# rtqichen/torchdiffeq

Measured on AMD Instinct MI355X. Metric: dopri5 RK-stages/sec at batch=65536x dim=128 (end-to-end adaptive trial steps incl. func, error norm, read-back and hos~, higher is better.
Workload: dtype f32; 1 GPU; BASELINE.json configs[1]: dopri5 adaptive, linear ODE dy/dt=Ay, batch=65536 x dim=128 fp32 per GPU, rtol=1e-7 atol=1e-9; global_batch=65536, rows_per_gpu=65536, dim=128, parallelism=batch-sharded x1, accepted=1937, rejected=2, lookahead=True, hip_graph=False

## Files before the change

### include/tdeq_hip.h

```cpp
#ifndef TDEQ_HIP_H
#define TDEQ_HIP_H

#include <stddef.h>
#include <stdint.h>

#ifdef __cplusplus
extern "C" {
#endif

#define TDEQ_ABI_VERSION 33
#define TDEQ_F32 0
#define TDEQ_F64 1
#define TDEQ_C64 2
#define TDEQ_C128 3
#define TDEQ_BF16 4
#define TDEQ_F16 5
#define TDEQ_MAX_TERMS 14
#define TDEQ_MAX_SUM_TERMS 8
#define TDEQ_MAX_DENSE_OUTPUTS 16
#define TDEQ_MAX_SEGMENTS 4096
#define TDEQ_INLINE_SEGMENTS 16
#define TDEQ_CHUNK_QUANTUM 1024

#define TDEQ_EINVAL (-1)
#define TDEQ_EWORKSPACE (-2)
// ... 78 lines not shown
int tdeq_stage_combine_multi_dev(const tdeq_multi_out* outs, int n_out, const void* y0, const void* acc_in,
                                 const void* const* k, int n_terms, const double* ctrl_dev, int64_t n, int dtype,
                                 void* stream);
int tdeq_stage_combine_multi_timed(const tdeq_multi_out* outs, int n_out, const void* y0, const void* acc_in,
                                   const void* const* k, int n_terms, double dt, int64_t n, int dtype, void* stream,
                                   void* start_event, void* stop_event);

int tdeq_error_norm_partial_ctrl(const void* err_partial, const void* y0, const void* y1, const void* const* k,
                                 const double* coef, int n_terms, double dt, const tdeq_segment* segs,
                                 const void* segs_dev, int n_seg, int64_t chunk, int64_t n_chunks, double* out_sumsq,
                                 double* out_nonfinite, const tdeq_step_ctrl* ctrl, double* out_ctrl, double* ctrl_dev,
                                 void* next_times, int state_in_dev, void* copy_last_k, void* workspace,
                                 size_t workspace_bytes, int dtype, void* stream);
int tdeq_stage_combine_sel(void* out, const void* y_acc, const void* f_acc, const void* y_rej, const void* f_rej,
                           double coef, const double* ctrl_dev, int64_t n, int dtype, void* stream);

int tdeq_step_controller(const double* sums, const double* nonfinite, const tdeq_segment* segs, const void* segs_dev,
                         int n_seg, double* out_sumsq, double* out_nonfinite, const tdeq_step_ctrl* ctrl,
                         double* out_ctrl, double* ctrl_dev, void* next_times, int state_in_dev, int dtype,
                         void* stream);

int tdeq_stage_combine_dev(void* out, void* err_out, const void* y0, const void* const* k, const double* coef,
                           const double* err_coef, int n_terms, const double* ctrl_dev, int64_t n, int dtype,
                           void* stream);
int tdeq_step_commit(void* y_prev, void* f_prev, void* y_cur, void* f_cur, const void* y1, const void* f1,
                     const double* ctrl_dev, int64_t n, int dtype, void* stream);

int tdeq_init_norms(int mode, const void* a, const void* b, const void* yscale,
                    const tdeq_segment* segs, const void* segs_dev, int n_seg, int64_t chunk,
                    int64_t n_chunks, double* out_sumsq, double* out_nonfinite, void* workspace, size_t workspace_bytes,
// ... 198 lines not shown
```

### torchdiffeq_amd/_native.py

```python
from __future__ import annotations

import contextlib
import ctypes
import functools
import math
import os
import threading
from typing import List, Optional, Sequence, Tuple

import numpy as np
import torch

TDEQ_ABI_VERSION = 33
TDEQ_F32, TDEQ_F64 = 0, 1
TDEQ_C64, TDEQ_C128 = 2, 3
TDEQ_BF16, TDEQ_F16 = 4, 5
TDEQ_MAX_TERMS = 14
TDEQ_INLINE_SEGMENTS = 16
TDEQ_CHUNK_QUANTUM = 1024
TDEQ_MAX_STAGE_TIMES = 16
TDEQ_MAX_DENSE_OUTPUTS = 16
TDEQ_MAX_MULTI_OUT = 4
TDEQ_MAX_GATHER = 4

_LIB_NAME = "libtdeq_hip.so"
_LIB_PATH = os.path.join(os.path.dirname(os.path.abspath(__file__)), _LIB_NAME)

_c_void_pp = ctypes.POINTER(ctypes.c_void_p)
# ... 104 lines not shown
                                                    ctypes.c_void_p, ctypes.c_int, ctypes.c_void_p, ctypes.c_void_p, ctypes.c_size_t,
                                                    ctypes.c_int, ctypes.c_void_p]),
    "tdeq_step_controller": (ctypes.c_int, [ctypes.c_void_p, ctypes.c_void_p, ctypes.POINTER(Segment), ctypes.c_void_p,
                                            ctypes.c_int, ctypes.c_void_p, ctypes.c_void_p,
                                            ctypes.POINTER(StepCtrl), ctypes.c_void_p, ctypes.c_void_p,
                                            ctypes.c_void_p, ctypes.c_int, ctypes.c_int, ctypes.c_void_p]),
    "tdeq_stage_combine_dev": (ctypes.c_int, [ctypes.c_void_p, ctypes.c_void_p, ctypes.c_void_p, _c_void_pp,
                                              _c_double_p, _c_double_p, ctypes.c_int, ctypes.c_void_p, ctypes.c_int64,
                                              ctypes.c_int, ctypes.c_void_p]),
    "tdeq_step_commit": (ctypes.c_int, [ctypes.c_void_p, ctypes.c_void_p, ctypes.c_void_p, ctypes.c_void_p,
                                        ctypes.c_void_p, ctypes.c_void_p, ctypes.c_void_p, ctypes.c_int64,
                                        ctypes.c_int, ctypes.c_void_p]),
    "tdeq_stage_combine_sel": (ctypes.c_int, [ctypes.c_void_p, ctypes.c_void_p, ctypes.c_void_p, ctypes.c_void_p,
                                              ctypes.c_void_p, ctypes.c_double, ctypes.c_void_p, ctypes.c_int64,
                                              ctypes.c_int, ctypes.c_void_p]),
    "tdeq_init_norms": (ctypes.c_int, [ctypes.c_int, ctypes.c_void_p, ctypes.c_void_p, ctypes.c_void_p,
                                       ctypes.POINTER(Segment), ctypes.c_void_p, ctypes.c_int,
                                       ctypes.c_int64, ctypes.c_int64, ctypes.c_void_p, ctypes.c_void_p,
                                       ctypes.c_void_p, ctypes.c_size_t, ctypes.c_int, ctypes.c_void_p]),
    "tdeq_init_scaled": (ctypes.c_int, [ctypes.c_int, ctypes.c_void_p, ctypes.c_void_p, ctypes.c_void_p,
                                        ctypes.POINTER(Segment), ctypes.c_void_p, ctypes.c_int, ctypes.c_int64,
                                        ctypes.c_int64, ctypes.c_void_p, ctypes.c_void_p, ctypes.c_int,
                                        ctypes.c_void_p]),
    "tdeq_dense_eval": (ctypes.c_int, [ctypes.c_void_p, ctypes.c_void_p, ctypes.c_void_p, ctypes.c_void_p,
                                       ctypes.c_void_p, _c_void_pp, _c_double_p, ctypes.c_int,
                                       ctypes.c_double, ctypes.c_double, ctypes.c_int64, ctypes.c_int,
                                       ctypes.c_void_p]),
    "tdeq_dense_eval_multi": (ctypes.c_int, [ctypes.c_void_p, ctypes.c_int64, ctypes.c_void_p, ctypes.c_void_p,
                                             ctypes.c_void_p, ctypes.c_void_p, _c_void_pp, _c_double_p, ctypes.c_int,
                                             ctypes.c_double, _c_double_p, ctypes.c_int, ctypes.c_int64, ctypes.c_int,
# ... 499 lines not shown
                                               dtype_code(y0.dtype), self._stream()), "tdeq_stage_combine_dev")

    def step_commit(self, y_prev, f_prev, y_cur, f_cur, y1, f1, plan: NormPlan) -> None:
        _check(self.lib.tdeq_step_commit(y_prev.data_ptr(), f_prev.data_ptr(), y_cur.data_ptr(), f_cur.data_ptr(),
                                         y1.data_ptr(), f1.data_ptr(), plan.ctrl_dev.data_ptr(), y_cur.numel(),
                                         dtype_code(y_cur.dtype), self._stream()), "tdeq_step_commit")

    def arm_readback(self, plan: NormPlan, n_sum: int = 1, ctrl: bool = True) -> None:
        self._arm(plan, n_sum, ctrl=ctrl)

    def stage_combine_sel(self, out, y_acc, f_acc, y_rej, f_rej, coef: float, plan: NormPlan) -> None:
        _check(self.lib.tdeq_stage_combine_sel(out.data_ptr(), y_acc.data_ptr(), f_acc.data_ptr(), y_rej.data_ptr(),
                                               f_rej.data_ptr(), coef, plan.ctrl_dev.data_ptr(), out.numel(),
                                               dtype_code(out.dtype), self._stream()), "tdeq_stage_combine_sel")

    def dense_eval(self, out, y0, y1, f0, f1, ks, coefs, dt: float, x: float) -> None:
        ptrs, cf, n = self._terms(ks, coefs)
        _check(self.lib.tdeq_dense_eval(out.data_ptr(), y0.data_ptr(), y1.data_ptr(), f0.data_ptr(),
                                        f1.data_ptr(), ptrs, cf, n, dt, x, y0.numel(),
                                        dtype_code(y0.dtype), self._stream()), "tdeq_dense_eval")

    def dense_eval_multi(self, out_rows, y0, y1, f0, f1, ks, coefs, dt: float, xs: Sequence[float]) -> None:
        ptrs, cf, n = self._terms(ks, coefs)
        m = len(xs)
        xa = (ctypes.c_double * m)(*xs)
        _check(self.lib.tdeq_dense_eval_multi(out_rows.data_ptr(), out_rows.stride(0) if m > 1 else y0.numel(),
                                              y0.data_ptr(), y1.data_ptr(), f0.data_ptr(), f1.data_ptr(), ptrs, cf, n,
                                              dt, xa, m, y0.numel(), dtype_code(y0.dtype), self._stream()),
               "tdeq_dense_eval_multi")

# ... 545 lines not shown
```

### torchdiffeq_amd/csrc/tdeq_abi.hip

```cpp
#include <hip/hip_runtime.h>
#include <hip/hip_ext.h>

#include <cstdlib>

#include "tdeq_kernels.hpp"
#include "tdeq_kernels_complex.hpp"
#include "tdeq_kernels_lp.hpp"

namespace {
using namespace tdeq;

constexpr int64_t kMaxGrid = 1 << 16;

inline unsigned stream_grid(int64_t n_items, int items_per_block) {
    int64_t g = (n_items + items_per_block - 1) / items_per_block;
    const int64_t cap = kMaxGrid;
    if (g > cap) g = cap;
    if (g < 1) g = 1;
    return (unsigned)g;
}

inline bool aligned16(const void* p) { return (reinterpret_cast<uintptr_t>(p) & 15u) == 0; }

inline int check_launch() {
// ... 530 lines not shown
    const bool vec = aligned16(out) && aligned16(y_acc) && aligned16(f_acc) && aligned16(y_rej) && aligned16(f_rej);
    if (vec) {
        const dim3 g(stream_grid(n / L, kBlock)), b(kBlock);
        switch (stream_policy((int64_t)3 * n * (int64_t)sizeof(T))) {
            case 1: hipLaunchKernelGGL((stage_combine_sel_kernel<T, true, 1>), g, b, 0, s, a); break;
            case 2: hipLaunchKernelGGL((stage_combine_sel_kernel<T, true, 2>), g, b, 0, s, a); break;
            case 3: hipLaunchKernelGGL((stage_combine_sel_kernel<T, true, 3>), g, b, 0, s, a); break;
            default: hipLaunchKernelGGL((stage_combine_sel_kernel<T, true, 0>), g, b, 0, s, a);
        }
    } else {
        hipLaunchKernelGGL((stage_combine_sel_kernel<T, false>), dim3(stream_grid(n, kBlock)), dim3(kBlock), 0, s, a);
    }
    return check_launch();
}

template <typename T>
int launch_init(int mode, const void* a_, const void* b_, const void* y_, const SegTable& st,
                double* out_sumsq, double* out_bad, double* ws, hipStream_t s) {
    InitArgs<T> a;
    a.a = static_cast<const T*>(a_);
    a.b = static_cast<const T*>(b_);
    a.y = static_cast<const T*>(y_);
    a.st = st;
    a.part0 = ws;
    a.part1 = ws + st.n_chunks;
    a.part_bad = ws + 2 * st.n_chunks;
    const bool vec = aligned16(a_) && aligned16(b_) && aligned16(y_);
    const dim3 g((unsigned)st.n_chunks), b(kBlock);
    if (mode == 0) {
        if (vec) hipLaunchKernelGGL((init_norms_kernel<T, 0, true>), g, b, 0, s, a);
// ... 777 lines not shown
    return dtype == TDEQ_F32 ? launch_commit<float>(y_prev, f_prev, y_cur, f_cur, y1, f1, ctrl_dev, n, s)
                             : launch_commit<double>(y_prev, f_prev, y_cur, f_cur, y1, f1, ctrl_dev, n, s);
}

int tdeq_stage_combine_sel(void* out, const void* y_acc, const void* f_acc, const void* y_rej, const void* f_rej,
                           double coef, const double* ctrl_dev, int64_t n, int dtype, void* stream) {
    if (!out || !y_acc || !f_acc || !y_rej || !f_rej || !ctrl_dev || n < 0 || (bad_dtype(dtype) && !lp_dtype(dtype))) return TDEQ_EINVAL;
    if (n == 0) return 0;
    hipStream_t s = static_cast<hipStream_t>(stream);
    if (dtype == TDEQ_BF16) return lp_launch_sel<lp::BF16>(out, y_acc, f_acc, y_rej, f_rej, coef, ctrl_dev, n, s);
    if (dtype == TDEQ_F16) return lp_launch_sel<lp::F16>(out, y_acc, f_acc, y_rej, f_rej, coef, ctrl_dev, n, s);
    return dtype == TDEQ_F32 ? launch_combine_sel<float>(out, y_acc, f_acc, y_rej, f_rej, coef, ctrl_dev, n, s)
                             : launch_combine_sel<double>(out, y_acc, f_acc, y_rej, f_rej, coef, ctrl_dev, n, s);
}

int tdeq_init_norms(int mode, const void* a, const void* b, const void* yscale, const tdeq_segment* segs,
                    const void* segs_dev, int n_seg, int64_t chunk, int64_t n_chunks, double* out_sumsq,
                    double* out_nonfinite, void* workspace, size_t workspace_bytes, int dtype,
                    void* stream) {
    if ((mode != 0 && mode != 1) || !a || !b || !yscale || !out_sumsq || !out_nonfinite || !workspace ||
        (bad_norm_dtype(dtype) && !lp_dtype(dtype)))
        return TDEQ_EINVAL;
    SegTable st;
    const int e = fill_segtable(st, segs, segs_dev, n_seg, chunk, n_chunks);
    if (e) return e;
    if (workspace_bytes < tdeq_workspace_bytes(n_chunks)) return TDEQ_EWORKSPACE;
    hipStream_t s = static_cast<hipStream_t>(stream);
    double* ws = static_cast<double*>(workspace);
    if (dtype == TDEQ_BF16) return lp_launch_init<lp::BF16>(mode, a, b, yscale, st, out_sumsq, out_nonfinite, ws, nullptr, nullptr, s);
    if (dtype == TDEQ_F16) return lp_launch_init<lp::F16>(mode, a, b, yscale, st, out_sumsq, out_nonfinite, ws, nullptr, nullptr, s);
// ... 323 lines not shown
```

### torchdiffeq_amd/csrc/tdeq_kernels.hpp

```cpp
#pragma once

#include <hip/hip_runtime.h>
#include <stdint.h>

#include "tdeq_hip.h"

namespace tdeq {

constexpr int kBlock = 256;
constexpr int kWave = 64;

typedef float f32x4 __attribute__((ext_vector_type(4)));
typedef double f64x2 __attribute__((ext_vector_type(2)));

template <typename T> struct VecOf;
template <> struct VecOf<float> { using type = f32x4; static constexpr int L = 4; };
template <> struct VecOf<double> { using type = f64x2; static constexpr int L = 2; };

template <typename V> __device__ __forceinline__ V vabs(V v);
template <> __device__ __forceinline__ f32x4 vabs(f32x4 v) {
    return f32x4{__builtin_fabsf(v.x), __builtin_fabsf(v.y), __builtin_fabsf(v.z), __builtin_fabsf(v.w)};
}
template <> __device__ __forceinline__ f64x2 vabs(f64x2 v) {
    return f64x2{__builtin_fabs(v.x), __builtin_fabs(v.y)};
// ... 230 lines not shown
            multi_elem<T, NT, E, POLICY, NOUTC, ACCC, DEVDT>(a, i);
    }
    if (VEC) {
        const int64_t t = ne * L + threadIdx.x;
        if (blockIdx.x == 0 && t < a.n) multi_elem<T, NT, T>(a, t);
    }
}

__device__ __forceinline__ double wave_sum(double v) {
#pragma unroll
    for (int off = kWave / 2; off > 0; off >>= 1) v += __shfl_down(v, off, kWave);
    return v;
}

template <int NV>
__device__ __forceinline__ void block_sum(double (&v)[NV], double* red) {
    const int lane = threadIdx.x & (kWave - 1);
    const int wave = threadIdx.x / kWave;
#pragma unroll
    for (int q = 0; q < NV; ++q) {
        v[q] = wave_sum(v[q]);
        if (lane == 0) red[q * (kBlock / kWave) + wave] = v[q];
    }
    __syncthreads();
    if (threadIdx.x == 0) {
#pragma unroll
        for (int q = 0; q < NV; ++q) {
            double s = red[q * (kBlock / kWave)];
#pragma unroll
            for (int w = 1; w < kBlock / kWave; ++w) s += red[q * (kBlock / kWave) + w];
            v[q] = s;
        }
    }
}

struct SegTable {
    tdeq_segment inl[TDEQ_INLINE_SEGMENTS];
    const tdeq_segment* dev;
    int n_seg;
    int64_t chunk;
    int64_t n_chunks;
};

__device__ __forceinline__ tdeq_segment get_segment(const SegTable& st, int s) {
    if (st.n_seg <= TDEQ_INLINE_SEGMENTS) return st.inl[s];
    return st.dev[s];
}

// ... 528 lines not shown
    float tt;
    if ((c.alpha_is_one >> i) & 1u) tt = ctl_prev16(t1T, tkind);
    else tt = ctl_rnd16(t0T + ctl_rnd16((float)c.alpha[i] * dtT, tkind), tkind);
    return ctl_bits16((float)c.time_sign * tt, tkind);
}

template <typename T>
__device__ __forceinline__ T ctl_stage_time(const tdeq_step_ctrl& c, double t0n, double dtn, int i) {
    const T t0T = (T)t0n, dtT = (T)dtn, t1T = (T)(t0n + dtn);
    T tt;
    if ((c.alpha_is_one >> i) & 1u) tt = ctl_prev(t1T);
    else tt = t0T + (T)c.alpha[i] * dtT;
    return (T)c.time_sign * tt;
}

constexpr int kCtrlInlineSegments = 4;
template <int NS>
__global__ __launch_bounds__(kBlock) void norm_finalize_ctrl_kernel(const CtrlArgs a) {
    __shared__ double red[2 * NS * (kBlock / kWave)];
    __shared__ double seg_val[2][NS];
    __shared__ double next_step[2];
    const int n_seg = a.st.n_seg;
    if (a.presummed) {
        const double* sums = a.in_sumsq ? a.in_sumsq : a.out_sumsq;
        if (a.in_sumsq)
            for (int s = threadIdx.x; s < n_seg; s += kBlock) {
                a.out_sumsq[s] = a.in_sumsq[s];
                a.out_bad[s] = a.in_bad[s];
            }
        double part[2] = {0.0, 0.0};
// ... 69 lines not shown
    if (threadIdx.x == 0) {
        const double dev_t0 = a.ctrl_dev[2], dev_dt = a.ctrl_dev[3];
        const double arg_t0 = c.t0, arg_dt = c.dt;
        const double step_t0 = a.state_in_dev ? dev_t0 : arg_t0;
        const double step_dt = a.state_in_dev ? dev_dt : arg_dt;
        double val = 0.0;
        if (a.presummed) val = seg_val[0][0];
        for (int s = 0; s < c.n_norm_seg && s < n_seg && !a.presummed; ++s) {
            const int64_t numel = a.st.inl[s].numel;
            if (numel == 0) continue;
            const double v = (s == 0 && numel == 1 && c.leading_abs && a.ratio_kind >= 2)
                                 ? (double)ctl_rnd16((float)seg_val[0][s], a.ratio_kind)
                                 : ctl_seg_norm(seg_val[0][s], numel, a.ratio_kind);
            val = ctl_nan_max(val, v);
        }
        const double ratio = a.ratio_kind == 1 ? (double)(float)val : val;
        bool accept = ratio <= 1.0;
        if (step_dt > c.max_step) accept = false;
        if (step_dt <= c.min_step) accept = true;
        double dt_next;
        if (ratio == 0.0) {
            dt_next = step_dt * c.ifactor;
        } else {
            const double dfactor = ratio < 1.0 ? 1.0 : c.dfactor;
            const double scaled = c.safety / pow(ratio, c.exponent);
            dt_next = step_dt * ctl_nan_min(c.ifactor, ctl_nan_max(scaled, dfactor));
        }
        dt_next = ctl_clamp(dt_next, c.min_step, c.max_step);
        const double t0n = accept ? step_t0 + step_dt : step_t0;
        double dtn = dt_next;
        if (!__builtin_isfinite(dtn)) dtn = c.min_step;
        dtn = ctl_clamp(dtn, c.min_step, c.max_step);
        a.ctrl_dev[0] = accept ? 1.0 : 0.0;
        a.ctrl_dev[1] = ctl_round_T(dtn, a.is_f32) * c.time_sign;
        a.ctrl_dev[2] = t0n;
        a.ctrl_dev[3] = dtn;
        next_step[0] = t0n;
        next_step[1] = dtn;
        a.out_ctrl[0] = accept ? 1.0 : 0.0;
        a.out_ctrl[1] = dt_next;
        a.out_ctrl[2] = ratio;
        a.out_ctrl[3] = t0n;
    }
    __syncthreads();
    const int i = threadIdx.x;
    if (i < c.n_times) {
        if (a.is_f32 >= 2) static_cast<uint16_t*>(a.next_times)[i] = ctl_stage_time16(c, next_step[0], next_step[1], i, a.is_f32);
        else if (a.is_f32) static_cast<float*>(a.next_times)[i] = ctl_stage_time<float>(c, next_step[0], next_step[1], i);
        else static_cast<double*>(a.next_times)[i] = ctl_stage_time<double>(c, next_step[0], next_step[1], i);
    }
    if (i < n_seg && !a.presummed) {
        a.out_sumsq[i] = seg_val[0][i];
        a.out_bad[i] = seg_val[1][i];
    }
}

template <typename T>
struct CombineDevArgs {
    T* out;
    T* err_out;
    const T* y0;
    const T* k[TDEQ_MAX_TERMS];
    T c[TDEQ_MAX_TERMS];
    T e[TDEQ_MAX_TERMS];
    int nt;
// ... 169 lines not shown
    const E* __restrict__ y = reinterpret_cast<const E*>(ys);
    const E* __restrict__ f = reinterpret_cast<const E*>(fs);
    if (i0 < ne) {
        if (!accept) {
            y_spec = ld_stream<POLICY>(y + i0);
            f_spec = ld_stream<POLICY>(f + i0);
        }
        st_stream<POLICY>(out + i0, y_spec + f_spec * c);
    }
    for (int64_t i = i0 + stride; i < ne; i += stride)
        st_stream<POLICY>(out + i, ld_stream<POLICY>(y + i) + ld_stream<POLICY>(f + i) * c);
    if (VEC) {
        const int64_t t = ne * L + threadIdx.x;
        if (blockIdx.x == 0 && t < a.n) a.out[t] = ys[t] + fs[t] * c;
    }
}

template <typename T, int NT>
struct DenseArgs {
    T* out;
    const T* y0;
    const T* y1;
    const T* f0;
    const T* f1;
    const T* k[NT];
    T c[NT];
    T dt;
    T x;
    int64_t n;
};
// ... 616 lines not shown
```

### torchdiffeq_amd/solvers/adaptive.py

```python
from __future__ import annotations

import bisect
import collections
import math
import os
import warnings
from typing import List, Optional, Sequence

import numpy as np
import torch

from .. import _native
from .._graph import (_AUTO_CAPTURE_AFTER_STEPS, _AUTO_MIN_GRID_STEPS, _GRAPH_AUTO_MAX_ELEMENTS,
                     _GRAPH_MODE_MAX_ELEMENTS, _CaptureFailed, _DtCell, _GraphStep, _capture, _graph_request,
                     _held_tensor_ptrs, _reusable_across_solves, _scalar_state, _side_effect_fingerprint, _side_stream,
                     _request_is_explicit, _stream_is_capturing, clear_graph_cache)
from .._scalars import is_low, power, rdiv, scalar_type
from ..autodiff import Ops, stitch
from ..misc import (BuiltinNorm, OdeFunc, Perturb, StateLayout, component_norm, find_event, handle_unused_kwargs, rms_norm,
                   vector_tolerances)
from ..misc import _null_callback as _null
from ..tableaus import (ADAPTIVE_HEUN, ADAPTIVE_TABLEAUS, BOSH3, CARRY_DEFAULT_ON, DOPRI5, DOPRI8, FEHLBERG2, FUSE_ODEINT, TSIT5, SparseRow,
                       Tableau, adams_coefficients, carry_plan, fused_lead, row_by_row_plan)
from ._common import _nan_max, _nan_min, _clamp, _norm_value, _as_float, optimal_step_size, optimal_step_size_in, _StepShadow, _NoShadow, _NO_SHADOW
from .events import AdaptiveEvents

STEP_CALLBACKS = ("callback_step", "callback_accept_step", "callback_reject_step")


class _LockStep:

    def __init__(self, group, replicated=()):
        import torch.distributed as dist
        self.dist = dist
        self.group = None if group is True else group
        self.replicated = sorted(set(int(i) for i in replicated))
        self.rank = dist.get_rank(self.group)
        backend = dist.get_backend(self.group)
        self.on_device = backend == "nccl"

# ... 183 lines not shown
            and func.time_dtype == y0.dtype and dist_sync is None
        device_ctrl = (getattr(self.kernels, "device_controller", True)
                       and (self._fuse is not None or self._whole_row_ctrl or self._vec_ctrl)
                       and (isinstance(self.norm, BuiltinNorm) or self._vec_ctrl)
                       and len(self._beta) <= _native.TDEQ_MAX_STAGE_TIMES and n_norm_seg >= 0
                       and self.step_t is None and self.jump_t is None and (self._sync is None or sync_dev)
                       and self._wide)
        self._plan_dev = self._plan_glob = None
        if device_ctrl and self._sync is not None:
            segs = self.layout.segments(rtol, atol)
            self._plan_dev = _native.NormPlan(segs, self.layout.total, self.layout.chunk, y0.device, pinned=False)
            self._plan_glob = self.kernels.make_plan([(off, gn, rt, at) for (off, _, rt, at), gn in
                                                      zip(segs, self._numels)], self.layout.total,
                                                     self.layout.chunk, y0.device)
        self._lookahead = device_ctrl and os.environ.get("TDEQ_LOOKAHEAD", "1") != "0"
        wanted, auto = _graph_request(hip_graph)
        self._graph_auto = auto
        self._graph_explicit = _request_is_explicit(hip_graph)
        if wanted and _stream_is_capturing():
            wanted = False
        self._graph_watch = wanted and auto and y0.device.type == "cuda"
        self._auto = None
        self._auto_steps = 0
        self._hold_pre = False
        self.hip_graph = wanted and device_ctrl and self._sync is None and y0.device.type == "cuda" \
            and (not self._vec_ctrl or getattr(self.kernels, "vec_ctrl_in_graph", False)) \
            and hasattr(self.kernels, "stage_combine_dev") \
            and self.layout.total <= (_GRAPH_AUTO_MAX_ELEMENTS if auto else _GRAPH_MODE_MAX_ELEMENTS) * \
            (2 if (y0.element_size() == 2 and not auto) else 1)
        if wanted and not auto and not self.hip_graph and hip_graph is not None:
# ... 473 lines not shown
        func, kern = self.func, self.kernels
        builtin_norm, vec_fused = self._partial_norm()
        ks, coefs = [k[j] for j in err_rem[0]], err_rem[1]
        vec_ctrl = self._vec_ctrl and not builtin_norm and (err_partial is None or vec_fused)
        if lookahead and ((err_partial is not None and (builtin_norm or vec_ctrl))
                          or (self._whole_row_ctrl and builtin_norm) or vec_ctrl):
            ctrl = self._ctrl
            ctrl.t0, ctrl.dt = t0, dt
            tnext = torch.empty(ctrl.n_times, dtype=func.time_dtype, device=y0.device)
            if vec_ctrl:
                kern.error_norm_vec_ctrl(self.plan, y0, y1, ks, coefs, dt_signed, self._vec_fused[0], self._vec_fused[1],
                                         ctrl, tnext, **({} if err_partial is None else {"partial": err_partial}))
            elif err_partial is None:
                kern.error_norm_ctrl(self.plan, y0, y1, ks, coefs, dt_signed, ctrl, tnext)
            elif self._sync is None:
                kern.error_norm_partial_ctrl(self.plan, err_partial, y0, y1, ks, coefs, dt_signed, ctrl, tnext)
            else:
                kern.error_norm_partial(self._plan_dev, err_partial, y0, y1, ks, coefs, dt_signed)
                self._sync.reduce_device(self._plan_dev.out, self.plan.n_seg)
                kern.step_controller(self.plan, self._plan_dev, self._plan_glob, ctrl, tnext, y0.dtype)
            if t1 < self._t_end and not self._hold_pre and not self._last_trial:
                yi_n = torch.empty_like(y0)
                kern.stage_combine_sel(yi_n, y1, k[-1], y0, f0, self._beta[0].coef[0], self.plan)
                tn = tnext.unbind(0)
                self._pre = (yi_n, tn, func.eval_at(tn[0], yi_n))
            accept_dev, dt_next_dev, error_ratio, bad = kern.read_ctrl(self.plan)
            return error_ratio, any(b != 0 for b in bad), (accept_dev, dt_next_dev)
        if not builtin_norm:
            return self._user_norm_ratio(y0, y1, k, dt_signed, err_partial, err_rem) + (None,)
        if err_partial is not None:
            kern.error_norm_partial(self.plan, err_partial, y0, y1, ks, coefs, dt_signed)
        else:
            kern.error_norm(self.plan, y0, y1, ks, coefs, dt_signed)
        sumsq, _, bad = self._read_norms()
        return self._segment_norm(sumsq, bad), any(b != 0 for b in bad), None

    def _commit(self, accept_step, dt_next, y0, y1, k, t0, dt, t1, dt_signed, dsh, dsh_signed, on_step_t, on_jump_t,
                y1_nonfinite) -> None:
        func = self.func
        if accept_step:
            if func.callback_accept_step is not _null:
                func.callback_accept_step(self._time_tensor(t0), y0, self._time_tensor(dt))
            rec = _DenseRecord(y0, y1, k, dt_signed, t0, t1, dsh_signed, self._anchor)
            if dsh is not None:
                clipped = on_step_t or on_jump_t
                self._anchor = None if clipped else (dsh if self._anchor is None else self._anchor + dsh)
                func.set_time_anchor(self._anchor)
            if on_step_t and self.next_step_index != len(self._step_t) - 1:
                self.next_step_index += 1
            f1 = k[-1]
# ... 109 lines not shown
```

Before: 17980 RK-stages/s.

## Fuse error norm, step controller and next-stage combine into one persistent kernel

Adds a single persistent-grid kernel that computes the error-norm partial sums, performs a grid-wide reduction through tagged atomic granules with spin-waiting, runs the step-size controller, and writes the selected next-stage input (accepted or rejected branch). This replaces the separate error_norm_partial_ctrl and stage_combine_sel launches and their extra passes over y0/y1/k. It is enabled automatically for large single-segment states. It relies on all workgroups being co-resident and falls back to the separate launches, with a warning, if a workgroup times out waiting.

Result: faster. 18410 RK-stages/s, median of 6 (+2.4%).

```diff
diff --git a/include/tdeq_hip.h b/include/tdeq_hip.h
--- a/include/tdeq_hip.h
+++ b/include/tdeq_hip.h
@@ -8,7 +8,7 @@
 extern "C" {
 #endif
 
-#define TDEQ_ABI_VERSION 33
+#define TDEQ_ABI_VERSION 34
 #define TDEQ_F32 0
 #define TDEQ_F64 1
 #define TDEQ_C64 2
@@ -117,6 +117,14 @@
                                  size_t workspace_bytes, int dtype, void* stream);
 int tdeq_stage_combine_sel(void* out, const void* y_acc, const void* f_acc, const void* y_rej, const void* f_rej,
                            double coef, const double* ctrl_dev, int64_t n, int dtype, void* stream);
+
+#define TDEQ_STEP_END_WORKSPACE_BYTES 8192
+int tdeq_step_end_fused(const void* err_partial, const void* y0, const void* y1, const void* const* k, const double* coef,
+                        int n_terms, double dt, const tdeq_segment* segs, int n_seg, int64_t chunk, int64_t n_chunks,
+                        double* out_sumsq, double* out_nonfinite, const tdeq_step_ctrl* ctrl, double* out_ctrl,
+                        double* ctrl_dev, void* next_times, void* out, const void* y_rej, const void* f_rej,
+                        double stage_coef, void* sync_workspace, size_t sync_workspace_bytes, int* status, int dtype,
+                        void* stream);
 
 int tdeq_step_controller(const double* sums, const double* nonfinite, const tdeq_segment* segs, const void* segs_dev,
                          int n_seg, double* out_sumsq, double* out_nonfinite, const tdeq_step_ctrl* ctrl,
diff --git a/torchdiffeq_amd/_native.py b/torchdiffeq_amd/_native.py
--- a/torchdiffeq_amd/_native.py
+++ b/torchdiffeq_amd/_native.py
@@ -11,7 +11,7 @@
 import numpy as np
 import torch
 
-TDEQ_ABI_VERSION = 33
+TDEQ_ABI_VERSION = 34
 TDEQ_F32, TDEQ_F64 = 0, 1
 TDEQ_C64, TDEQ_C128 = 2, 3
 TDEQ_BF16, TDEQ_F16 = 4, 5
@@ -146,6 +146,13 @@
     "tdeq_stage_combine_sel": (ctypes.c_int, [ctypes.c_void_p, ctypes.c_void_p, ctypes.c_void_p, ctypes.c_void_p,
                                               ctypes.c_void_p, ctypes.c_double, ctypes.c_void_p, ctypes.c_int64,
                                               ctypes.c_int, ctypes.c_void_p]),
+    "tdeq_step_end_fused": (ctypes.c_int, [ctypes.c_void_p, ctypes.c_void_p, ctypes.c_void_p, _c_void_pp, _c_double_p,
+                                           ctypes.c_int, ctypes.c_double, ctypes.POINTER(Segment), ctypes.c_int,
+                                           ctypes.c_int64, ctypes.c_int64, ctypes.c_void_p, ctypes.c_void_p,
+                                           ctypes.POINTER(StepCtrl), ctypes.c_void_p, ctypes.c_void_p, ctypes.c_void_p,
+                                           ctypes.c_void_p, ctypes.c_void_p, ctypes.c_void_p, ctypes.c_double,
+                                           ctypes.c_void_p, ctypes.c_size_t, ctypes.c_void_p, ctypes.c_int,
+                                           ctypes.c_void_p]),
     "tdeq_init_norms": (ctypes.c_int, [ctypes.c_int, ctypes.c_void_p, ctypes.c_void_p, ctypes.c_void_p,
                                        ctypes.POINTER(Segment), ctypes.c_void_p, ctypes.c_int,
                                        ctypes.c_int64, ctypes.c_int64, ctypes.c_void_p, ctypes.c_void_p,
@@ -675,6 +682,50 @@
                                                f_rej.data_ptr(), coef, plan.ctrl_dev.data_ptr(), out.numel(),
                                                dtype_code(out.dtype), self._stream()), "tdeq_stage_combine_sel")
 
+    step_end_fused_capable = True
+    STEP_END_WORKSPACE_BYTES = 8192
+
+    def step_end_fused(self, plan: NormPlan, err_partial, y0, y1, ks, coefs, dt: float, ctrl: StepCtrl, next_times,
+                       out, y_rej, f_rej, stage_coef: float) -> bool:
+        if getattr(plan, "step_end_ws", None) is None:
+            plan.step_end_ws = torch.zeros(self.STEP_END_WORKSPACE_BYTES // 8, dtype=torch.int64, device=y0.device)
+            plan.step_end_status = torch.zeros(4, dtype=torch.int32, device="cpu", pin_memory=True)
+            plan.step_end_status_np = plan.step_end_status.numpy()
+        n = len(ks)
+        ptrs = (ctypes.c_void_p * max(n, 1))(*[k.data_ptr() for k in ks])
+        cf = (ctypes.c_double * max(n, 1))(*coefs)
+        self._arm(plan, 1, ctrl=True)
+        rc = self.lib.tdeq_step_end_fused(
+            err_partial.data_ptr(), y0.data_ptr(), y1.data_ptr(), ptrs, cf, n, dt, plan.segs, plan.n_seg, plan.chunk,
+            plan.n_chunks, plan.out_ptr, plan.bad_ptr, ctypes.byref(ctrl), plan.ctrl_ptr, plan.ctrl_dev.data_ptr(),
+            next_times.data_ptr(), out.data_ptr(), y_rej.data_ptr(), f_rej.data_ptr(), stage_coef,
+            plan.step_end_ws.data_ptr(), self.STEP_END_WORKSPACE_BYTES, plan.step_end_status.data_ptr(),
+            dtype_code(y0.dtype), self._stream())
+        if rc in (-1, -2):
+            plan.expect = ()
+            return False
+        _check(rc, "tdeq_step_end_fused")
+        return True
+
+    def read_ctrl_fused(self, plan: NormPlan):
+        status = plan.step_end_status_np
+        if plan.pinned and self._mode == "poll" and plan.expect:
+            bits, sent = plan.out_bits, self._SENTINEL
+            (a0, a1), (b0, b1) = plan.expect
+            spins = 0
+            while ((bits[a0:a1] == sent).any() or (bits[b0:b1] == sent).any()) and status[0] == 0:
+                spins += 1
+                if spins & 0xFFFFF == 0:
+                    torch.cuda.current_stream().synchronize()
+                    break
+        else:
+            torch.cuda.current_stream().synchronize()
+        if status[0] != 0:
+            torch.cuda.current_stream().synchronize()
+            plan.expect = ()
+            return None
+        return self.read_ctrl(plan)
+
     def dense_eval(self, out, y0, y1, f0, f1, ks, coefs, dt: float, x: float) -> None:
         ptrs, cf, n = self._terms(ks, coefs)
         _check(self.lib.tdeq_dense_eval(out.data_ptr(), y0.data_ptr(), y1.data_ptr(), f0.data_ptr(),
diff --git a/torchdiffeq_amd/csrc/tdeq_abi.hip b/torchdiffeq_amd/csrc/tdeq_abi.hip
--- a/torchdiffeq_amd/csrc/tdeq_abi.hip
+++ b/torchdiffeq_amd/csrc/tdeq_abi.hip
@@ -568,6 +568,74 @@
     return check_launch();
 }
 
+constexpr long long kEndSpinTicks = 400000;
+
+inline int device_cu_count() {
+    int dev = 0, cus = 0;
+    if (hipGetDevice(&dev) != hipSuccess) return 0;
+    if (hipDeviceGetAttribute(&cus, hipDeviceAttributeMultiprocessorCount, dev) != hipSuccess) return 0;
+    return cus;
+}
+
+template <typename T>
+int step_end_geometry(const SegTable& st, const void* const* ptrs, int n_ptrs, int& vpl) {
+    constexpr int L = VecOf<T>::L;
+    if (st.n_seg != 1 || st.inl[0].chunk_start != 0) return TDEQ_EINVAL;
+    const int64_t numel = st.inl[0].numel;
+    if (numel < L || numel % L != 0 || numel > st.chunk * st.n_chunks) return TDEQ_EINVAL;
+    if (st.n_chunks != (numel + st.chunk - 1) / st.chunk) return TDEQ_EINVAL;
+    if (st.chunk % (L * kBlock) != 0) return TDEQ_EINVAL;
+    vpl = (int)(st.chunk / (L * kBlock));
+    if (vpl != 1 && vpl != 2) return TDEQ_EINVAL;
+    const int64_t capacity = (int64_t)kEndGrid * kEndQuarters * (kEndVecs / vpl);
+    if (st.n_chunks > capacity) return TDEQ_EINVAL;
+    for (int q = 0; q < n_ptrs; ++q) if (!aligned16(ptrs[q])) return TDEQ_EINVAL;
+    return 0;
+}
+
+template <typename T>
+int launch_step_end(const void* partial, const void* y0, const void* y1, const void* k_last, double coef_err, double dt,
+                    const SegTable& st, double* out_sumsq, double* out_bad, const tdeq_step_ctrl* ctrl, double* out_ctrl,
+                    double* ctrl_dev, void* next_times, void* out, const void* y_rej, const void* f_rej, double coef,
+                    void* sync_ws, int* status, hipStream_t s) {
+    const void* ptrs[7] = {partial, y0, y1, k_last, out, y_rej, f_rej};
+    int vpl = 0;
+    const int e = step_end_geometry<T>(st, ptrs, 7, vpl);
+    if (e) return e;
+    static const int cus = device_cu_count();
+    if (cus < kEndGrid) return TDEQ_EINVAL;
+    StepEndArgs<T> a;
+    a.partial = static_cast<const T*>(partial);
+    a.y0 = static_cast<const T*>(y0);
+    a.y1 = static_cast<const T*>(y1);
+    a.k_last = static_cast<const T*>(k_last);
+    a.c_err = (T)coef_err * (T)dt;
+    a.numel = st.inl[0].numel;
+    a.chunk = st.chunk;
+    a.n_chunks = st.n_chunks;
+    a.rtol = st.inl[0].rtol;
+    a.atol = st.inl[0].atol;
+    a.c = *ctrl;
+    a.tkind = sizeof(T) == 4 ? 1 : 0;
+    a.out_sumsq = out_sumsq;
+    a.out_bad = out_bad;
+    a.out_ctrl = out_ctrl;
+    a.ctrl_dev = ctrl_dev;
+    a.next_times = next_times;
+    a.out = static_cast<T*>(out);
+    a.y_rej = static_cast<const T*>(y_rej);
+    a.f_rej = static_cast<const T*>(f_rej);
+    a.coef = (T)coef;
+    a.granules = static_cast<unsigned long long*>(sync_ws);
+    a.ticket = reinterpret_cast<unsigned*>(a.granules + kEndGrid * kEndGranules);
+    a.status = status;
+    a.spin_ticks = kEndSpinTicks;
+    const dim3 g(kEndGrid), b(kEndBlock);
+    if (vpl == 2) hipLaunchKernelGGL((step_end_fused_kernel<T, 2>), g, b, 0, s, a);
+    else hipLaunchKernelGGL((step_end_fused_kernel<T, 1>), g, b, 0, s, a);
+    return check_launch();
+}
+
 template <typename T>
 int launch_init(int mode, const void* a_, const void* b_, const void* y_, const SegTable& st,
                 double* out_sumsq, double* out_bad, double* ws, hipStream_t s) {
@@ -1375,6 +1443,31 @@
                              : launch_combine_sel<double>(out, y_acc, f_acc, y_rej, f_rej, coef, ctrl_dev, n, s);
 }
 
+int tdeq_step_end_fused(const void* err_partial, const void* y0, const void* y1, const void* const* k, const double* coef,
+                        int n_terms, double dt, const tdeq_segment* segs, int n_seg, int64_t chunk, int64_t n_chunks,
+                        double* out_sumsq, double* out_nonfinite, const tdeq_step_ctrl* ctrl, double* out_ctrl,
+                        double* ctrl_dev, void* next_times, void* out, const void* y_rej, const void* f_rej,
+                        double stage_coef, void* sync_workspace, size_t sync_workspace_bytes, int* status, int dtype,
+                        void* stream) {
+    if (!err_partial || !y0 || !y1 || !k || !coef || n_terms != 1 || !k[0] || !segs || bad_dtype(dtype)) return TDEQ_EINVAL;
+    if (!out_sumsq || !out_nonfinite || !ctrl || !out_ctrl || !ctrl_dev || !next_times) return TDEQ_EINVAL;
+    if (!out || !y_rej || !f_rej || !sync_workspace || !status) return TDEQ_EINVAL;
+    if (ctrl->n_times < 1 || ctrl->n_times > TDEQ_MAX_STAGE_TIMES || ctrl->n_norm_seg < 0 || ctrl->n_norm_seg > n_seg)
+        return TDEQ_EINVAL;
+    if (out == err_partial || out == y0 || out == y1 || out == k[0] || out == y_rej || out == f_rej) return TDEQ_EINVAL;
+    if (n_seg != 1) return TDEQ_EINVAL;
+    SegTable st;
+    const int e = fill_segtable(st, segs, nullptr, n_seg, chunk, n_chunks);
+    if (e) return e;
+    if (sync_workspace_bytes < TDEQ_STEP_END_WORKSPACE_BYTES || !aligned16(sync_workspace)) return TDEQ_EWORKSPACE;
+    hipStream_t s = static_cast<hipStream_t>(stream);
+    return dtype == TDEQ_F32
+               ? launch_step_end<float>(err_partial, y0, y1, k[0], coef[0], dt, st, out_sumsq, out_nonfinite, ctrl, out_ctrl,
+                                        ctrl_dev, next_times, out, y_rej, f_rej, stage_coef, sync_workspace, status, s)
+               : launch_step_end<double>(err_partial, y0, y1, k[0], coef[0], dt, st, out_sumsq, out_nonfinite, ctrl, out_ctrl,
+                                         ctrl_dev, next_times, out, y_rej, f_rej, stage_coef, sync_workspace, status, s);
+}
+
 int tdeq_init_norms(int mode, const void* a, const void* b, const void* yscale, const tdeq_segment* segs,
                     const void* segs_dev, int n_seg, int64_t chunk, int64_t n_chunks, double* out_sumsq,
                     double* out_nonfinite, void* workspace, size_t workspace_bytes, int dtype,
diff --git a/torchdiffeq_amd/csrc/tdeq_kernels.hpp b/torchdiffeq_amd/csrc/tdeq_kernels.hpp
--- a/torchdiffeq_amd/csrc/tdeq_kernels.hpp
+++ b/torchdiffeq_amd/csrc/tdeq_kernels.hpp
@@ -268,24 +268,29 @@
 }
 
 template <int NV>
-__device__ __forceinline__ void block_sum(double (&v)[NV], double* red) {
+__device__ __forceinline__ void block_sum_stage(double (&v)[NV], double* red, int wave) {
     const int lane = threadIdx.x & (kWave - 1);
-    const int wave = threadIdx.x / kWave;
 #pragma unroll
     for (int q = 0; q < NV; ++q) {
         v[q] = wave_sum(v[q]);
         if (lane == 0) red[q * (kBlock / kWave) + wave] = v[q];
     }
+}
+template <int NV>
+__device__ __forceinline__ void block_sum_finish(double (&v)[NV], const double* red) {
+#pragma unroll
+    for (int q = 0; q < NV; ++q) {
+        double s = red[q * (kBlock / kWave)];
+#pragma unroll
+        for (int w = 1; w < kBlock / kWave; ++w) s += red[q * (kBlock / kWave) + w];
+        v[q] = s;
+    }
+}
+template <int NV>
+__device__ __forceinline__ void block_sum(double (&v)[NV], double* red) {
+    block_sum_stage<NV>(v, red, threadIdx.x / kWave);
     __syncthreads();
-    if (threadIdx.x == 0) {
-#pragma unroll
-        for (int q = 0; q < NV; ++q) {
-            double s = red[q * (kBlock / kWave)];
-#pragma unroll
-            for (int w = 1; w < kBlock / kWave; ++w) s += red[q * (kBlock / kWave) + w];
-            v[q] = s;
-        }
-    }
+    if (threadIdx.x == 0) block_sum_finish<NV>(v, red);
 }
 
 struct SegTable {
@@ -844,6 +849,53 @@
     return (T)c.time_sign * tt;
 }
 
+struct CtlDecision {
+    bool accept;
+    double dt_next;
+    double ratio;
+    double t0n;
+    double dtn;
+};
+__device__ __forceinline__ CtlDecision ctl_decide(const tdeq_step_ctrl& c, double val, int ratio_kind, double step_t0,
+                                                  double step_dt) {
+    CtlDecision d;
+    d.ratio = ratio_kind == 1 ? (double)(float)val : val;
+    d.accept = d.ratio <= 1.0;
+    if (step_dt > c.max_step) d.accept = false;
+    if (step_dt <= c.min_step) d.accept = true;
+    double dt_next;
+    if (d.ratio == 0.0) {
+        dt_next = step_dt * c.ifactor;
+    } else {
+        const double dfactor = d.ratio < 1.0 ? 1.0 : c.dfactor;
+        const double scaled = c.safety / pow(d.ratio, c.exponent);
+        dt_next = step_dt * ctl_nan_min(c.ifactor, ctl_nan_max(scaled, dfactor));
+    }
+    d.dt_next = ctl_clamp(dt_next, c.min_step, c.max_step);
+    d.t0n = d.accept ? step_t0 + step_dt : step_t0;
+    double dtn = d.dt_next;
+    if (!__builtin_isfinite(dtn)) dtn = c.min_step;
+    d.dtn = ctl_clamp(dtn, c.min_step, c.max_step);
+    return d;
+}
+__device__ __forceinline__ void ctl_write_words(const CtlDecision& d, const tdeq_step_ctrl& c, int tkind, double* ctrl_dev,
+                                                double* out_ctrl) {
+    ctrl_dev[0] = d.accept ? 1.0 : 0.0;
+    ctrl_dev[1] = ctl_round_T(d.dtn, tkind) * c.time_sign;
+    ctrl_dev[2] = d.t0n;
+    ctrl_dev[3] = d.dtn;
+    out_ctrl[0] = d.accept ? 1.0 : 0.0;
+    out_ctrl[1] = d.dt_next;
+    out_ctrl[2] = d.ratio;
+    out_ctrl[3] = d.t0n;
+}
+__device__ __forceinline__ void ctl_write_stage_time(const tdeq_step_ctrl& c, void* next_times, double t0n, double dtn, int i,
+                                                     int tkind) {
+    if (tkind >= 2) static_cast<uint16_t*>(next_times)[i] = ctl_stage_time16(c, t0n, dtn, i, tkind);
+    else if (tkind) static_cast<float*>(next_times)[i] = ctl_stage_time<float>(c, t0n, dtn, i);
+    else static_cast<double*>(next_times)[i] = ctl_stage_time<double>(c, t0n, dtn, i);
+}
+
 constexpr int kCtrlInlineSegments = 4;
 template <int NS>
 __global__ __launch_bounds__(kBlock) void norm_finalize_ctrl_kernel(const CtrlArgs a) {
@@ -943,41 +995,14 @@
                                  : ctl_seg_norm(seg_val[0][s], numel, a.ratio_kind);
             val = ctl_nan_max(val, v);
         }
-        const double ratio = a.ratio_kind == 1 ? (double)(float)val : val;
-        bool accept = ratio <= 1.0;
-        if (step_dt > c.max_step) accept = false;
-        if (step_dt <= c.min_step) accept = true;
-        double dt_next;
-        if (ratio == 0.0) {
-            dt_next = step_dt * c.ifactor;
-        } else {
-            const double dfactor = ratio < 1.0 ? 1.0 : c.dfactor;
-            const double scaled = c.safety / pow(ratio, c.exponent);
-            dt_next = step_dt * ctl_nan_min(c.ifactor, ctl_nan_max(scaled, dfactor));
-        }
-        dt_next = ctl_clamp(dt_next, c.min_step, c.max_step);
-        const double t0n = accept ? step_t0 + step_dt : step_t0;
-        double dtn = dt_next;
-        if (!__builtin_isfinite(dtn)) dtn = c.min_step;
-        dtn = ctl_clamp(dtn, c.min_step, c.max_step);
-        a.ctrl_dev[0] = accept ? 1.0 : 0.0;
-        a.ctrl_dev[1] = ctl_round_T(dtn, a.is_f32) * c.time_sign;
-        a.ctrl_dev[2] = t0n;
-        a.ctrl_dev[3] = dtn;
-        next_step[0] = t0n;
-        next_step[1] = dtn;
-        a.out_ctrl[0] = accept ? 1.0 : 0.0;
-        a.out_ctrl[1] = dt_next;
-        a.out_ctrl[2] = ratio;
-        a.out_ctrl[3] = t0n;
+        const CtlDecision d = ctl_decide(c, val, a.ratio_kind, step_t0, step_dt);
+        ctl_write_words(d, c, a.is_f32, a.ctrl_dev, a.out_ctrl);
+        next_step[0] = d.t0n;
+        next_step[1] = d.dtn;
     }
     __syncthreads();
     const int i = threadIdx.x;
-    if (i < c.n_times) {
-        if (a.is_f32 >= 2) static_cast<uint16_t*>(a.next_times)[i] = ctl_stage_time16(c, next_step[0], next_step[1], i, a.is_f32);
-        else if (a.is_f32) static_cast<float*>(a.next_times)[i] = ctl_stage_time<float>(c, next_step[0], next_step[1], i);
-        else static_cast<double*>(a.next_times)[i] = ctl_stage_time<double>(c, next_step[0], next_step[1], i);
-    }
+    if (i < c.n_times) ctl_write_stage_time(c, a.next_times, next_step[0], next_step[1], i, a.is_f32);
     if (i < n_seg && !a.presummed) {
         a.out_sumsq[i] = seg_val[0][i];
         a.out_bad[i] = seg_val[1][i];
@@ -1177,6 +1202,225 @@
         const int64_t t = ne * L + threadIdx.x;
         if (blockIdx.x == 0 && t < a.n) a.out[t] = ys[t] + fs[t] * c;
     }
+}
+
+constexpr int kEndGrid = 256;
+constexpr int kEndBlock = 1024;
+constexpr int kEndQuarters = kEndBlock / kBlock;
+constexpr int kEndVecs = 8;
+constexpr int kEndGranules = 3;
+constexpr unsigned kEndTagBit = 0x80000000u;
+
+template <typename T>
+struct StepEndArgs {
+    const T* partial;
+    const T* y0;
+    const T* y1;
+    const T* k_last;
+    T c_err;
+    int64_t numel;
+    int64_t chunk;
+    int64_t n_chunks;
+    double rtol;
+    double atol;
+    tdeq_step_ctrl c;
+    int tkind;
+    double* out_sumsq;
+    double* out_bad;
+    double* out_ctrl;
+    double* ctrl_dev;
+    void* next_times;
+    T* out;
+    const T* y_rej;
+    const T* f_rej;
+    T coef;
+    unsigned long long* granules;
+    unsigned* ticket;
+    int* status;
+    long long spin_ticks;
+};
+
+template <typename T, int VPL>
+__global__ __launch_bounds__(kEndBlock) void step_end_fused_kernel(const StepEndArgs<T> a) {
+    using V = typename VecOf<T>::type;
+    constexpr int L = VecOf<T>::L;
+    constexpr int R = kEndVecs / VPL;
+    constexpr int NW = kBlock / kWave;
+    __shared__ double red[R * kEndQuarters][2 * NW];
+    __shared__ double csum[R * kEndQuarters][2];
+    __shared__ double fin[2 * NW];
+    __shared__ double bcast[2];
+    __shared__ unsigned s_epoch;
+    __shared__ int s_fail;
+    const int tid = threadIdx.x;
+    const int quarter = __builtin_amdgcn_readfirstlane(tid / kBlock), qt = tid % kBlock;
+    const int64_t w = blockIdx.x;
+    const T rtol = (T)a.rtol, atol = (T)a.atol;
+    auto at = [](const T* p, unsigned index) -> const V* {
+        return reinterpret_cast<const V*>(reinterpret_cast<const char*>(p) + (size_t)(index * 16u));
+    };
+    const int vchunk = (int)(a.chunk / L);
+    auto slot = [&](int r, int u, unsigned& index) -> bool {
+        const int64_t b = w + (int64_t)kEndGrid * (r * kEndQuarters + quarter);
+        int64_t valid = a.numel - b * a.chunk;
+        valid = valid < 0 ? 0 : (valid > a.chunk ? a.chunk : valid);
+        const int nv = (int)(valid / L);
+        const unsigned first = nv > 0 ? (unsigned)((int)b * vchunk) : 0u, last = nv > 0 ? (unsigned)(nv - 1) : 0u;
+        const unsigned i = (unsigned)(qt + u * kBlock);
+        index = first + (i < last ? i : last);
+        return i < (unsigned)nv;
+    };
+    V ry1[R][VPL], rk[R][VPL];
+#pragma unroll
+    for (int r = 0; r < R; ++r)
+#pragma unroll
+        for (int u = 0; u < VPL; ++u) {
+            unsigned i;
+            slot(r, u, i);
+            ry1[r][u] = *at(a.y1, i);
+            rk[r][u] = *at(a.k_last, i);
+        }
+    constexpr bool PRE = VPL == 1;
+    constexpr int PB = PRE ? 1 : 0;
+    constexpr int G = VPL > 2 ? 2 : VPL;
+    V re[PB + 1][G], r0[PB + 1][G];
+    auto stage = [&](int r, int u0) {
+#pragma unroll
+        for (int g = 0; g < G; ++g) {
+            unsigned i;
+            slot(r, u0 + g, i);
+            re[r & PB][g] = *at(a.partial, i);
+            r0[r & PB][g] = *at(a.y0, i);
+        }
+    };
+    stage(0, 0);
+    unsigned my_ticket = 0;
+    if (tid == 0) {
+        s_fail = 0;
+        my_ticket = __hip_atomic_fetch_add(a.ticket, 1u, __ATOMIC_RELAXED, __HIP_MEMORY_SCOPE_AGENT);
+    }
+#pragma unroll
+    for (int r = 0; r < R; ++r) {
+        if (PRE && r + 1 < R) stage(r + 1, 0);
+        double acc[2] = {0.0, 0.0};
+#pragma unroll
+        for (int u0 = 0; u0 < VPL; u0 += G) {
+            if (!PRE && (r > 0 || u0 > 0)) stage(r, u0);
+#pragma unroll
+            for (int g = 0; g < G; ++g) {
+                const int u = u0 + g;
+                unsigned i;
+                const bool ok = slot(r, u, i);
+                const V e = re[r & PB][g] + rk[r][u] * a.c_err;
+                double t0 = acc[0], t1 = acc[1];
+#pragma unroll
+                for (int q = 0; q < L; ++q) {
+                    tol_accumulate<T>(e[q], r0[r & PB][g][q], ry1[r][u][q], rtol, atol, t0, t1);
+                    if constexpr (sizeof(T) == 8) __builtin_amdgcn_sched_barrier(0);
+                }
+                acc[0] = ok ? t0 : acc[0];
+                acc[1] = ok ? t1 : acc[1];
+            }
+            if (!PRE) __builtin_amdgcn_sched_barrier(0);
+        }
+        block_sum_stage<2>(acc, red[r * kEndQuarters + quarter], qt / kWave);
+        __builtin_amdgcn_sched_barrier(0);
+    }
+    if (tid == 0) s_epoch = (my_ticket / kEndGrid) | kEndTagBit;
+    __syncthreads();
+    const unsigned epoch = s_epoch;
+    if (tid < R * kEndQuarters) {
+        double cs[2];
+        block_sum_finish<2>(cs, red[tid]);
+        csum[tid][0] = cs[0];
+        csum[tid][1] = cs[1];
+    }
+    __builtin_amdgcn_fence(__ATOMIC_RELEASE, "workgroup");
+    __builtin_amdgcn_wave_barrier();
+    __builtin_amdgcn_fence(__ATOMIC_ACQUIRE, "workgroup");
+    if (tid == 0) {
+        const int mine = w < a.n_chunks ? (int)((a.n_chunks - w + kEndGrid - 1) / kEndGrid) : 0;
+        double a0 = 0.0, a1 = 0.0;
+#pragma unroll 4
+        for (int j = 0; j < mine; ++j) {
+            a0 += csum[j][0];
+            a1 += csum[j][1];
+        }
+        const unsigned long long bits = (unsigned long long)__double_as_longlong(a0);
+        const unsigned long long tag = (unsigned long long)epoch << 32;
+        unsigned long long* g = a.granules + w * kEndGranules;
+        __hip_atomic_store(g + 0, tag | (bits & 0xffffffffull), __ATOMIC_RELAXED, __HIP_MEMORY_SCOPE_AGENT);
+        __hip_atomic_store(g + 1, tag | (bits >> 32), __ATOMIC_RELAXED, __HIP_MEMORY_SCOPE_AGENT);
+        __hip_atomic_store(g + 2, tag | (unsigned long long)(unsigned)a1, __ATOMIC_RELAXED, __HIP_MEMORY_SCOPE_AGENT);
+    }
+    if (tid < kEndGrid) {
+        const unsigned long long* g = a.granules + (int64_t)tid * kEndGranules;
+        const long long t_start = wall_clock64();
+        unsigned long long x0, x1, x2;
+        bool failed = false;
+        for (;;) {
+            x0 = __hip_atomic_load(g + 0, __ATOMIC_RELAXED, __HIP_MEMORY_SCOPE_AGENT);
+            x1 = __hip_atomic_load(g + 1, __ATOMIC_RELAXED, __HIP_MEMORY_SCOPE_AGENT);
+            x2 = __hip_atomic_load(g + 2, __ATOMIC_RELAXED, __HIP_MEMORY_SCOPE_AGENT);
+            const bool have = (unsigned)(x0 >> 32) == epoch && (unsigned)(x1 >> 32) == epoch && (unsigned)(x2 >> 32) == epoch;
+            if (__all(have)) break;
+            if (wall_clock64() - t_start > a.spin_ticks) {
+                failed = true;
+                break;
+            }
+            __builtin_amdgcn_s_sleep(2);
+        }
+        if (failed) s_fail = 1;
+        double acc[2];
+        acc[0] = __longlong_as_double((long long)(((x1 & 0xffffffffull) << 32) | (x0 & 0xffffffffull)));
+        acc[1] = (double)(unsigned)(x2 & 0xffffffffull);
+        block_sum_stage<2>(acc, fin, tid / kWave);
+    }
+    __syncthreads();
+    if (s_fail) {
+        if (tid == 0) *a.status = 1;
+        return;
+    }
+    const tdeq_step_ctrl& c = a.c;
+    if (tid == 0) {
+        double tot[2];
+        block_sum_finish<2>(tot, fin);
+        double val = 0.0;
+        if (c.n_norm_seg > 0 && a.numel != 0) val = ctl_nan_max(val, ctl_seg_norm(tot[0], a.numel, a.tkind));
+        *const_cast<volatile double*>(&bcast[0]) = val;
+        val = *const_cast<volatile double*>(&bcast[0]);
+        const CtlDecision d = ctl_decide(c, val, a.tkind, c.t0, c.dt);
+        bcast[0] = d.accept ? 1.0 : 0.0;
+        bcast[1] = ctl_round_T(d.dtn, a.tkind) * c.time_sign;
+        if (w == 0) {
+            ctl_write_words(d, c, a.tkind, a.ctrl_dev, a.out_ctrl);
+            a.out_sumsq[0] = tot[0];
+            a.out_bad[0] = tot[1];
+#pragma unroll 1
+            for (int i = 0; i < c.n_times; ++i) ctl_write_stage_time(c, a.next_times, d.t0n, d.dtn, i, a.tkind);
+        }
+    }
+    __syncthreads();
+    const bool accept = bcast[0] != 0.0;
+    const T cs = a.coef * (T)bcast[1];
+    if (!accept) {
+#pragma unroll
+        for (int r = 0; r < R; ++r)
+#pragma unroll
+            for (int u = 0; u < VPL; ++u) {
+                unsigned i;
+                slot(r, u, i);
+                ry1[r][u] = *at(a.y_rej, i);
+                rk[r][u] = *at(a.f_rej, i);
+            }
+    }
+#pragma unroll
+    for (int r = 0; r < R; ++r)
+#pragma unroll
+        for (int u = 0; u < VPL; ++u) {
+            unsigned i;
+            if (slot(r, u, i)) *const_cast<V*>(at(a.out, i)) = ry1[r][u] + rk[r][u] * cs;
+        }
 }
 
 template <typename T, int NT>
diff --git a/torchdiffeq_amd/solvers/adaptive.py b/torchdiffeq_amd/solvers/adaptive.py
--- a/torchdiffeq_amd/solvers/adaptive.py
+++ b/torchdiffeq_amd/solvers/adaptive.py
@@ -24,6 +24,9 @@
                        Tableau, adams_coefficients, carry_plan, fused_lead, row_by_row_plan)
 from ._common import _nan_max, _nan_min, _clamp, _norm_value, _as_float, optimal_step_size, optimal_step_size_in, _StepShadow, _NoShadow, _NO_SHADOW
 from .events import AdaptiveEvents
+
+STEP_END_AUTO_FROM = 3 << 21
+_STEP_END_OFF = False
 
 STEP_CALLBACKS = ("callback_step", "callback_accept_step", "callback_reject_step")
 
@@ -237,6 +240,11 @@
                                                       zip(segs, self._numels)], self.layout.total,
                                                      self.layout.chunk, y0.device)
         self._lookahead = device_ctrl and os.environ.get("TDEQ_LOOKAHEAD", "1") != "0"
+        se_env = os.environ.get("TDEQ_STEP_END", "auto").lower()
+        self._step_end = (self._lookahead and se_env != "0" and self._sync is None and self.layout.n_seg == 1
+                          and self._fuse is not None and not self._vec_ctrl and isinstance(self.norm, BuiltinNorm)
+                          and getattr(self.kernels, "step_end_fused_capable", False)
+                          and (se_env == "1" or self.layout.total >= STEP_END_AUTO_FROM))
         wanted, auto = _graph_request(hip_graph)
         self._graph_auto = auto
         self._graph_explicit = _request_is_explicit(hip_graph)
@@ -740,6 +748,11 @@
             elif err_partial is None:
                 kern.error_norm_ctrl(self.plan, y0, y1, ks, coefs, dt_signed, ctrl, tnext)
             elif self._sync is None:
+                if self._step_end and not _STEP_END_OFF and len(ks) == 1 and ks[0] is k[-1] \
+                        and t1 < self._t_end and not self._hold_pre and not self._last_trial:
+                    decided = self._step_end_fused(y0, f0, y1, ks, coefs, err_partial, dt_signed, ctrl, tnext)
+                    if decided is not None:
+                        return decided
                 kern.error_norm_partial_ctrl(self.plan, err_partial, y0, y1, ks, coefs, dt_signed, ctrl, tnext)
             else:
                 kern.error_norm_partial(self._plan_dev, err_partial, y0, y1, ks, coefs, dt_signed)
@@ -760,6 +773,30 @@
             kern.error_norm(self.plan, y0, y1, ks, coefs, dt_signed)
         sumsq, _, bad = self._read_norms()
         return self._segment_norm(sumsq, bad), any(b != 0 for b in bad), None
+
+    def _step_end_fused(self, y0, f0, y1, ks, coefs, err_partial, dt_signed, ctrl, tnext):
+        global _STEP_END_OFF
+        func, kern = self.func, self.kernels
+        yi_n = torch.empty_like(y0)
+        if not kern.step_end_fused(self.plan, err_partial, y0, y1, ks, coefs, dt_signed, ctrl, tnext, yi_n, y0, f0,
+                                   self._beta[0].coef[0]):
+            self._step_end = False
+            return None
+        tn = tnext.unbind(0)
+        nfe = getattr(func, "nfe", None)
+        self._pre = (yi_n, tn, func.eval_at(tn[0], yi_n))
+        read = kern.read_ctrl_fused(self.plan)
+        if read is None:
+            _STEP_END_OFF = True
+            warnings.warn("tdeq_step_end_fused: a workgroup gave up waiting for the others (the device is shared, or not "
+                          "all 256 workgroups were resident); this step end is redone with the separate launches and "
+                          "the fused launch stays off for this process", RuntimeWarning)
+            self._pre = None
+            if nfe is not None:
+                func.nfe = nfe
+            return None
+        accept_dev, dt_next_dev, error_ratio, bad = read
+        return error_ratio, any(b != 0 for b in bad), (accept_dev, dt_next_dev)
 
     def _commit(self, accept_step, dt_next, y0, y1, k, t0, dt, t1, dt_signed, dsh, dsh_signed, on_step_t, on_jump_t,
                 y1_nonfinite) -> None:
```
